# cgmb/euler

Hardware: AMD Instinct MI355X
Metric: cells*steps/sec of sim_step() (frames incl. the PCG pressure projection) + pressure-solve HBM GB/s vs roofline (higher is better)
Workload: dtype f64

## Files before the change

### euler_amd/csrc/driver.hip

```cpp
#include "euler_dev.h"
#include "k_mg.h"

#include <math.h>
#include <stdarg.h>
#include <stdlib.h>
#include <string.h>

#include <vector>

int eu_launch_build_system(euler_sim* S, float dt);
int eu_launch_velocity_update(euler_sim* S, float dt, int finish);
int eu_pressure_current(euler_sim* S);
int eu_unskew(euler_sim* S, const void* skew, void* rowmajor, int elem_bytes);
int eu_unskew_fluid(euler_sim* S, const double* skew, double* rowmajor);
double* eu_current_search_direction(euler_sim* S);
int eu_launch_tile_table(euler_sim* S);
int eu_skew(euler_sim* S, const void* rowmajor, void* skew, int elem_bytes);
int eu_set_source_count(euler_sim* S, size_t nsrc);

static thread_local char g_err[512] = "";

void eu_set_error(const char* fmt, ...) {
  va_list ap;
  va_start(ap, fmt);
// ... 105 lines not shown
  S->tile_w = w;
  return EULER_OK;
}

bool eu_resident_eligible(const euler_sim* S) {
  if (S->res_disabled || S->cfg.resident == EULER_RESIDENT_OFF) return false;
  if (S->cfg.precond != EULER_PRECOND_IC0_TILE || S->tile_w != 16 || S->cfg.sweep_mode == EULER_SWEEP_SIMPLE || S->cfg.dot_mode != EULER_DOT_TREE) return false;
  if (S->has_comm || S->slab_on || S->p2p_on) return false;
  const int cap = eu_resident_capacity(const_cast<euler_sim*>(S), S->cfg.pcg_precision == EULER_PCG_F32);
  if (S->cfg.pcg_precision == EULER_PCG_F32) return cap > 0 && S->geom.nbands * (S->geom.T / 16) <= 4 * cap;
  return cap > 0;
}
extern "C" int euler_resident_info(euler_sim* S, uint64_t out[3]) {
  if (!S || !out) return EULER_EINVAL;
  out[0] = eu_resident_eligible(S) ? 1 : 0; out[1] = S->res_solves; out[2] = S->res_fallbacks;
  return EULER_OK;
}

extern "C" int euler_set_option(euler_sim* S, int32_t key, int64_t value) {
  if (!S || key <= 0 || key >= EULER_OPT__COUNT) { eu_set_error("euler_set_option: unknown key %d", (int)key); return EULER_EINVAL; }
  bool ok = true;
  const char* when = nullptr;
  switch (key) {
    case EULER_OPT_P_STEPS: ok = value == 2 || value == 4 || value == 8; break;
    case EULER_OPT_SA_RUN: ok = value == 8 || value == 16 || value == 32;
      if (ok && value != 8 && (S->has_comm || eu_is_two_level(S))) when = "on a handle without a communicator, in the parity or the plain tile-local mode (the others run runs of 8)";
      break;
    case EULER_OPT_RCCL_SMALL: ok = value >= 0 && value <= 2; if (S->rccl) when = "before euler_set_comm_rccl"; break;
    case EULER_OPT_RCCL_NO_EXCHANGE: ok = value == 0 || value == 1; if (S->rccl) when = "before euler_set_comm_rccl"; break;
    case EULER_OPT_SLAB_FUSION: ok = value == 0 || value == 1; if (S->p2p_on) when = "before euler_p2p_connect"; break;
    case EULER_OPT_RESIDENT_CAP: case EULER_OPT_GRID4_MIN_CELLS: case EULER_OPT_RESIDENT_FORCE_TIMEOUT: ok = value >= 0; break;
    case EULER_OPT_MG_SPLIT_LEVEL: ok = value >= -1 && value < 12; break;
    case EULER_OPT_PROFILE_STRIDE: ok = value >= 1 && value <= 1024; break;
    case EULER_OPT_MG_SPLIT_ACTIVE: ok = false; break;
    case EULER_OPT_ADVECT_RK2: ok = value == 0 || value == 1;
      if (ok && value == 1 && S->slab_on) when = "on a whole-grid handle (row slabs: the midpoint samples reach one row beyond the ghost rows)";
      break;
    case EULER_OPT_ADVECT_MACCORMACK: ok = value == 0 || value == 1;
      if (ok && value == 1 && S->slab_on) when = "on a whole-grid handle (row slabs: the correction reads the forward result one row beyond the own rows)";
      break;
    default: ok = value == 0 || value == 1; break;
  }
  if (!ok) { eu_set_error("euler_set_option: key %d does not take the value %lld", (int)key, (long long)value); return EULER_EINVAL; }
  if (when) { eu_set_error("euler_set_option: key %d must be set %s", (int)key, when); return EULER_ESTATE; }
  HIPCHK(hipStreamSynchronize(S->stream));
  if (key == EULER_OPT_ADVECT_MACCORMACK && value == 1 && !S->mc_u) {
    float *a = nullptr, *b = nullptr;
    const size_t bytes = S->C * sizeof(float);
    if (eu_dalloc(S, &a, S->C, EU_MEM_HANDLE, EU_MEM_ZERO | EU_DEV_QUIET) || eu_dalloc(S, &b, S->C, EU_MEM_HANDLE, EU_MEM_ZERO | EU_DEV_QUIET)) {
      (void)eu_dev_free(S, a);
      eu_set_error("euler_set_option: EULER_OPT_ADVECT_MACCORMACK needs %zu bytes of scratch", 2 * bytes);
      return EULER_ENOMEM;
    }
    S->mc_u = a; S->mc_v = b;
  }
  if (key == EULER_OPT_P_STEPS || key == EULER_OPT_SA_RUN) {
    int rcp = eu_pressure_current(S);
    if (rcp) return rcp;
  }
  S->opt[key] = value;
  if (key == EULER_OPT_P_STEPS || key == EULER_OPT_SA_RUN) S->s_ring_n = 0;
  if (key == EULER_OPT_MG_SPLIT_LEVEL) { eu_mg_split_release(S); S->opt[EULER_OPT_MG_SPLIT_ACTIVE] = 0; }
  return EULER_OK;
}
extern "C" int euler_get_option(euler_sim* S, int32_t key, int64_t* value) {
  if (!S || !value || key <= 0 || key >= EULER_OPT__COUNT) { eu_set_error("euler_get_option: unknown key %d", (int)key); return EULER_EINVAL; }
  *value = S->opt[key];
  return EULER_OK;
}

static const char* eu_precond_combination(const euler_sim* S, int precond, int tile_w, int has_comm, int slab_on, int p2p_on) {
  const bool coarse = precond == EULER_PRECOND_IC0_TILE2 || precond == EULER_PRECOND_IC0_TILE_MG;
  if (!coarse) return nullptr;
  if (tile_w != 16 || S->cfg.sweep_mode == EULER_SWEEP_SIMPLE) return "the coarse-correction preconditioners run on tiles of 16 records with the band schedule";
  if (precond == EULER_PRECOND_IC0_TILE2 && (has_comm || slab_on)) return "EULER_PRECOND_IC0_TILE2 runs on one GPU (row slabs: EULER_PRECOND_IC0_TILE_MG)";
  if (precond == EULER_PRECOND_IC0_TILE_MG && has_comm && (!slab_on || p2p_on)) return "EULER_PRECOND_IC0_TILE_MG with several ranks: row-slab handles without mailboxes only";
  return nullptr;
}

extern "C" int euler_set_precond(euler_sim* S, int32_t precond, int32_t tile_records) {
  if (!S || precond < EULER_PRECOND_IC0 || precond > EULER_PRECOND_IC0_TILE_MG) { eu_set_error("euler_set_precond: bad argument"); return EULER_EINVAL; }
  const int w = tile_records <= 0 ? 16 : tile_records;
  if (w != 8 && w != 16 && w != 32) { eu_set_error("precond_tile_records = %d: 8, 16 or 32 (0 = 16)", tile_records); return EULER_EINVAL; }
  if (const char* why = eu_precond_combination(S, precond, w, S->has_comm, S->slab_on, S->p2p_on)) { eu_set_error("euler_set_precond: %s", why); return EULER_EINVAL; }
// ... 882 lines not shown
```

### euler_amd/csrc/euler_dev.h

```cpp
#pragma once

#include <hip/hip_runtime.h>
#include <stdint.h>
#include <stdio.h>

#include "euler.h"
#include "euler_host.h"
#include "eu_valid.h"
#include "eu_mem.h"

#define EU_H 1.0f
#define EU_RHO 1.0f
#define EU_G (-10.0f)

#define CM_FLUID 0x01
#define CM_RIGHT 0x02
#define CM_UP    0x04
#define CM_LEFT  0x08
#define CM_DOWN  0x10
#define CM_DIAG_SHIFT 5
#define CM_INTERIOR 0x9F
#define EU_CHUNK_INTERIOR 0x80000000u

enum {
  KC_TIMESTEP = 0, KC_MARKER_ADVECT, KC_MARKER_EVENTS, KC_MARKER_BIN, KC_MARKER_COMPACT, KC_SOURCES,
  KC_SELECT, KC_EXTRAPOLATE, KC_ADVECT_VELOCITY, KC_BUILD_SYSTEM, KC_PRECON_FACTOR,
  KC_FORWARD_SOLVE, KC_BACKWARD_SOLVE, KC_APPLY_A, KC_DOT, KC_UPDATE_PR, KC_UPDATE_SEARCH,
  KC_REDUCE_FINAL, KC_VELOCITY_UPDATE, KC_JACOBI, KC_MISC, KC_PRECOND_TILE, KC_COARSE_CYCLE, KC_RESIDENT, KC__COUNT
};

struct PcgScalars {
  double sigma, zs, sigma_new, alpha, beta, rnorm;
// ... 160 lines not shown
  double* cc_null;
  int mg_levels, mg_nx[12], mg_ny[12];
  size_t mg_off[12], mg_cells;
  double* mg_a;
  unsigned long long* mg_a0i;
  double *mg_rhs, *mg_x;
  double* mg_wd;
  uint8_t* mg_inner0; double mg_ic[9];
  double* mg_part;
  double* mg_dot;
  double* mg_null0;
  double* mg_m0;
  void* mg_split;
  double* mg_xbuf; int mg_xslot;
  unsigned long long* res_gran;
  unsigned long long res_tag;
  int* res_err;
  int res_disabled;
  unsigned int res_last_chunks;
  int res_have_last, res_skip_once;
  unsigned long long res_solves, res_fallbacks;
  int pcg_fields_resident;
  int tile_w;
  double* s_ring[8];
  void* s_ring_alloc[8];
  double* s_base[2];
  int s_ring_n;
  int s_launched;
  int s_none;
  int s_stale;
  const double* tile_as_override;
  double* partial2;
  struct RngJump* rng_jump;
  uint8_t* chunk_flag;
  uint8_t* chunk_prev;
  uint8_t* chunk_part;
  eu_mem mem;
  double* zhalo;
  double* zrows;
  int z_halo_last;
  double* tile_table;
  unsigned long long* chunk_bits;
  unsigned int* chunk_list;
  size_t chunk_words, chunk_cap;
  double* xrows;
  size_t xrow_len;
  int gs_cur;
  double* alpha_buf;
// ... 311 lines not shown
```

### euler_amd/csrc/k_grid.hip

```cpp
#include "k_pcg.h"
#include "k_transport.h"

#include <stdlib.h>

__device__ __forceinline__ void dt_from_maxima(MarkerState* ms, float frame_time_left, unsigned int mu_bits, unsigned int mv_bits) {
  const float mu = __uint_as_float(mu_bits), mv = __uint_as_float(mv_bits);
  const float max_distance = 0.75f * EU_H;
  const float max_velocity = sqrtf(mu + mv);
  ms->dt = fminf(max_distance / max_velocity, frame_time_left);
  ms->max_u2_bits = 0u;
  ms->max_v2_bits = 0u;
}
template <bool FUSE_DT>
__global__ __launch_bounds__(256) void k_maxsq(const float* __restrict__ u, const float* __restrict__ v,
                                               int X, int Y, MarkerState* ms, int y0, int y1, float frame_time_left) {
  float mu = 0.f, mv = 0.f;
  const bool vec = (X & 3) == 0;
  for (int yq = y0 + 4 * (int)blockIdx.x; yq < y1; yq += 4 * (int)gridDim.x) {
    if (vec) {
      for (int x = 4 * (int)threadIdx.x; x < X; x += 4 * 256) {
        float4 a[4], b[4];
#pragma unroll
        for (int r = 0; r < 4; ++r) {
          const int y = yq + r < y1 ? yq + r : y1 - 1;
// ... 651 lines not shown
    const bool f1 = count[i + 1] != 0;
    float o = 0.f;
    if (solid[i] | solid[i + 1]) o = 0.f;
    else if (f0 | f1) {
      double p1 = p[skew_index(g, x + 1, y)];
      if (f1 && p1 < 0.0) p1 = 0.0;
      o = uin[i] + (neg_inv * (float)(p1 - p0)) * dt;
    }
    uout[i] = o;
  }
  if (y < Y - 1) {
    const bool f1 = count[i + X] != 0;
    float o = 0.f;
    if (solid[i] | solid[i + X]) o = 0.f;
    else if (f0 | f1) {
      double p1 = p[skew_index(g, x, y + 1)];
      if (f1 && p1 < 0.0) p1 = 0.0;
      o = vin[i] + (neg_inv * (float)(p1 - p0)) * dt;
    }
    vout[i] = o;
  }
}

struct VuRing { const double* s[8]; int n, steps, use; };
#define VU_W 48
#define VU_ILP 4
__global__ __launch_bounds__(256) void k_velocity_update_para(const float* __restrict__ uin, const float* __restrict__ vin, float* __restrict__ uout, float* __restrict__ vout,
                                                              const double* __restrict__ p, const uint8_t* __restrict__ mask, const uint8_t* __restrict__ count,
                                                              const uint8_t* __restrict__ solid, SkewGeom g, float dt, const PcgScalars* sc, VuRing ring, MarkerState* ms,
                                                              int band_lo, int do_max, int skip_zero,
                                                              const uint8_t* __restrict__ tmap, int tnx) {
  __shared__ double sp[65][VU_W + 1];
  __shared__ float s_mu[4], s_mv[4];
  const int units = g.T / VU_W;
  const size_t blk = eu_xcd_block();
  const int band = band_lo + (int)(blk / units), t0 = (int)(blk % units) * VU_W;
  const int X = g.X, Y = g.Y, tid = threadIdx.x;
  if (skip_zero && tmap && eu_tiles_idle_cur(tmap, tnx, band, t0 > 63 ? (t0 - 63) >> 6 : 0, (t0 + VU_W - 1) >> 6, true)) return;
  int cnt = 0, from = 0;
  if (ring.use && sc->nonzero && sc->iters > 0) {
    const int n_it = sc->iters;
    from = n_it - 1 >= ring.steps ? (n_it - 1) / ring.steps * ring.steps : 0;
    cnt = n_it - from;
  }
  double al[8];
  const double* sq[8];
#pragma unroll
  for (int j = 0; j < 8; ++j) { const int it = from + (j < cnt ? j : 0); al[j] = sc->alpha_hist[it & 7]; sq[j] = ring.s[it % ring.n]; }
  const size_t ebase = ((size_t)band * g.TS + (size_t)t0) * 64;
  static_assert((64 * VU_W) % (256 * VU_ILP) == 0, "whole rounds of VU_ILP elements per thread");
  for (int c0 = tid; c0 < 64 * VU_W; c0 += 256 * VU_ILP) {
    uint8_t m[VU_ILP];
    double pv[VU_ILP];
    bool any = false;
#pragma unroll
    for (int u = 0; u < VU_ILP; ++u) { m[u] = mask[ebase + (size_t)(c0 + 256 * u)]; any = any || (m[u] & CM_FLUID); }
    if (__any(any)) {
#pragma unroll
      for (int u = 0; u < VU_ILP; ++u) pv[u] = p[ebase + (size_t)(c0 + 256 * u)];
#pragma unroll
      for (int j = 0; j < 8; ++j)
        if (j < cnt) {
          double sv[VU_ILP];
#pragma unroll
          for (int u = 0; u < VU_ILP; ++u) sv[u] = sq[j][ebase + (size_t)(c0 + 256 * u)];
#pragma unroll
          for (int u = 0; u < VU_ILP; ++u) pv[u] = pv[u] + sv[u] * al[j];
        }
    } else {
#pragma unroll
      for (int u = 0; u < VU_ILP; ++u) pv[u] = 0.0;
    }
#pragma unroll
    for (int u = 0; u < VU_ILP; ++u) {
      const int c = c0 + 256 * u;
      const double v = (m[u] & CM_FLUID) ? (pv[u] < 0.0 ? 0.0 : pv[u]) : 0.0;
      sp[(c & 127) >> 1][2 * (c >> 7) + (c & 1)] = v;
    }
  }
  {
    size_t e = 0;
    bool want = false, above = false;
    int hl = 0, hj = 0;
    if (tid < 64) { e = ebase + (size_t)VU_W * 64 + 2 * (size_t)tid; want = true; hl = tid; hj = VU_W; }
    else if (tid < 64 + VU_W) {
      const int j = tid - 64 + 1, x = t0 - 64 + j;
      hl = 64; hj = j;
      if (x >= 0 && x < X && band + 1 < g.nbands && count[(size_t)(band + 1) * 64 * X + x] != 0) { e = ((size_t)(band + 1) * g.TS + (size_t)(x & ~1)) * 64 + (size_t)(x & 1); want = true; above = true; }
    }
    if (tid < 64 + VU_W) {
      double pv = 0.0;
      if (want && (above || (mask[e] & CM_FLUID))) {
        pv = p[e];
#pragma unroll
        for (int j = 0; j < 8; ++j) if (j < cnt) pv = pv + sq[j][e] * al[j];
        pv = pv < 0.0 ? 0.0 : pv;
      }
      sp[hl][hj] = pv;
    }
  }
  __syncthreads();
  const float neg_inv = -(1.f / (EU_RHO * EU_H));
  float mu = 0.f, mv = 0.f;
  static_assert((64 * VU_W) % (256 * 4) == 0, "whole rounds of four cells per thread");
  for (int c0 = tid; c0 < 64 * VU_W; c0 += 256 * 4) {
    size_t ii[4]; bool in[4]; int ll[4], jj[4], xx[4], yy[4];
    uint8_t c_0[4], c_r[4], c_u[4], s_0[4], s_r[4], s_u[4];
    float ui[4], vi[4];
#pragma unroll
    for (int u = 0; u < 4; ++u) {
      const int c = c0 + 256 * u;
      ll[u] = c / VU_W; jj[u] = c % VU_W;
      xx[u] = t0 - ll[u] + jj[u]; yy[u] = band * 64 + ll[u];
      in[u] = xx[u] >= 0 && xx[u] < X && yy[u] < Y;
      ii[u] = (size_t)(yy[u] < Y ? yy[u] : Y - 1) * X + (size_t)(xx[u] < 0 ? 0 : xx[u] >= X ? X - 1 : xx[u]);
      const bool hr = in[u] && xx[u] < X - 1, hu = in[u] && yy[u] < Y - 1;
      c_0[u] = count[ii[u]]; s_0[u] = solid[ii[u]];
      c_r[u] = count[ii[u] + (hr ? 1 : 0)]; s_r[u] = solid[ii[u] + (hr ? 1 : 0)];
// ... 90 lines not shown
           S->solid, S->b, S->r, S->p, S->q, S->z, S->cellmask, S->sc, S->geom, dt, S->e_lo, S->e_cnt, S->chunk_flag, S->chunk_part, S->chunk_prev);
  eu_vd_assembled(&S->vd);
  LAUNCH(S, KC_BUILD_SYSTEM, k_pack_chunk_bits, dim3(eu_blocks(S->chunk_words, 256)), dim3(256), S->chunk_flag, S->chunk_bits, S->chunk_words, S->chunk_cap);
  int rc = eu_ordered_select(S, S->chunk_bits, S->chunk_words, S->chunk_list, &S->sc->n_chunks);
  if (rc) return rc;
  const bool no_interior = S->opt[EULER_OPT_NO_INTERIOR] != 0;
  if (!no_interior)
    LAUNCH(S, KC_BUILD_SYSTEM, k_mark_interior, dim3(eu_blocks(S->chunk_cap, 256)), dim3(256), S->chunk_list, S->sc, S->chunk_part);
  return eu_launch_band_ranges(S);
}

int eu_pressure_current(euler_sim* S) {
  const int mode = eu_vd_pressure_owes(&S->vd);
  if (!mode) return EULER_OK;
  eu_vd_pressure_made_current(&S->vd);
  if (mode == 1) { int rc = eu_launch_finish_p(S); if (rc) return rc; }
  LAUNCH(S, KC_VELOCITY_UPDATE, k_clamp_p, dim3(eu_blocks(S->e_cnt, 256 * 4, 4096)), dim3(256), S->p, S->cellmask, S->e_lo, S->e_cnt);
  return EULER_OK;
}
int eu_launch_velocity_update(euler_sim* S, float dt, int finish) {
  const bool one_pass = (!S->has_comm || S->slab_on) && S->opt[EULER_OPT_VELOCITY_TWO_PASS] == 0 && (!S->slab_on || !finish);
  if (one_pass) {
    VuRing ring;
    for (int k = 0; k < 8; ++k) ring.s[k] = S->s_ring[k < S->s_ring_n ? k : 0];
    ring.n = S->s_ring_n > 0 ? S->s_ring_n : 1; ring.steps = ring.n; ring.use = finish && S->s_ring_n > 0;
    if (!ring.use) for (int k = 0; k < 8; ++k) ring.s[k] = S->p;
    const int do_max = S->slab_on ? 0 : 1;
    if (eu_vd_update_clears_maxima(&S->vd, do_max)) HIPCHK(hipMemsetAsync(&S->ms->max_u2_bits, 0, 2 * sizeof(unsigned int), S->stream));
    LAUNCH(S, KC_VELOCITY_UPDATE, k_velocity_update_para, dim3((unsigned)((size_t)(S->band_hi - S->band_lo) * (S->geom.T / VU_W))), dim3(256), S->utmp, S->vtmp, S->u, S->v, S->p, S->cellmask,
           S->count, S->solid, S->geom, dt, S->sc, ring, S->ms, S->band_lo, do_max, eu_vd_update_skips_zeros(&S->vd, S->slab_on),
           eu_tile_map_on(S) ? (const uint8_t*)S->tmap : (const uint8_t*)nullptr, S->tmap_nx);
    eu_vd_velocity_updated(&S->vd, 1, ring.use, do_max);
    return EULER_OK;
  }
  if (finish) { int rc = eu_launch_finish_p(S); if (rc) return rc; }
  dim3 grid((S->X + 63) / 64, (S->row_hi - S->row_lo + 3) / 4);
  LAUNCH(S, KC_VELOCITY_UPDATE, k_velocity_update, grid, dim3(256), S->utmp, S->vtmp, S->u, S->v, S->p, S->count,
         S->solid, S->geom, dt, S->row_lo, S->row_hi);
  eu_vd_velocity_updated(&S->vd, 0, 0, 0);
  return EULER_OK;
}

template <typename T>
__global__ __launch_bounds__(256) void k_unskew(const T* __restrict__ skew, T* __restrict__ rowmajor, SkewGeom g, int y0, int y1) {
  const size_t i = (size_t)blockIdx.x * blockDim.x + threadIdx.x;
  if (i < (size_t)g.X * (y1 - y0)) rowmajor[i] = skew[skew_index(g, (int)(i % g.X), y0 + (int)(i / g.X))];
}
template <typename T>
__global__ __launch_bounds__(256) void k_skew(const T* __restrict__ rowmajor, T* __restrict__ skew, SkewGeom g, int y0, int y1) {
// ... 28 lines not shown
```

### euler_amd/csrc/k_pcg.h

```cpp
#pragma once

#include "euler_dev.h"
#include "k_mg.h"

#define COMM_CALL(expr) do { if ((expr) != 0) { eu_set_error("communicator callback failed: %s", #expr); return EULER_ECOMM; } } while (0)
#define LOC(ptr) ((ptr) + S->e_lo)
enum { SW_FACTOR = 0, SW_FORWARD = 1, SW_BACKWARD = 2 };

int eu_launch_build_system(euler_sim* S, float dt);
int eu_launch_velocity_update(euler_sim* S, float dt, int finish);
int eu_launch_band_ranges(euler_sim* S);
int eu_launch_sweep(euler_sim* S, int op, int cls, int force, int fin_qq = -1);
int eu_launch_factor_tile(euler_sim* S, int force);
int eu_launch_precond_tile(euler_sim* S, int rupd, int sweeps, int fin_dot, int force, double alpha, bool r_only = false, int zform = -1);
int eu_launch_search_apply(euler_sim* S, int it);
int eu_launch_finish_p(euler_sim* S);
int eu_launch_dot(euler_sim* S, const double* a, const double* b, int fin_op, int force);
int eu_comm_exchange(euler_sim* S, double* send_lo, double* send_hi, double* recv_lo, double* recv_hi, int count, double* small, int nsmall);
int eu_comm_finish(euler_sim* S, int fin_op, int is_max, int force);
int eu_comm_halo_two(euler_sim* S, double* a, double* b);
bool tile_recompute(const euler_sim* S);
int p_steps(const euler_sim* S);

enum { FIN_SIGMA_INIT = 0, FIN_ALPHA, FIN_RNORM, FIN_BETA, FIN_STORE_ONLY, FIN_TO_COMM };
// ... 125 lines not shown
    const double qv = t * cpre;
    const double res = (cm & CM_FLUID) ? qv : 0.0;
    const double carry = -1.0 * cpre * res;
    own = carry; out = carry;
    if (j & 1) zz[j >> 1].y = res; else zz[j >> 1].x = res;
  }
  own = 0.0; out = 0.0;
#pragma unroll
  for (int j = W - 1; j >= 0; --j) {
    const int cm = (int)((mm[j >> 1] >> ((j & 1) * 8)) & 0xff);
    const double cin = (j & 1) ? zz[j >> 1].y : zz[j >> 1].x, cpre = (j & 1) ? pp[j >> 1].y : pp[j >> 1].x;
    const double nbv = wave_shift_inject<DPP_WAVE_SHL1>(out, 0.0);
    const double kr = ((cm & CM_RIGHT) ? -1.0 : 0.0) * cpre, ku = ((cm & CM_UP) ? -1.0 : 0.0) * cpre;
    const double t = cin - kr * own - ku * nbv;
    const double zv = t * cpre;
    const double res = (cm & CM_FLUID) ? zv : 0.0;
    own = res; out = res;
    if (DOT && (cm & CM_FLUID)) dsum += res * ((j & 1) ? rr[j >> 1].y : rr[j >> 1].x);
    if (j & 1) zz[j >> 1].y = res; else zz[j >> 1].x = res;
  }
}
struct ZrArgs { const double* r; const double* pre; const double* table; const double* halo; const double* rows; int X; };
struct CoarseRef { const double* y; int shift, nx, ny, band0; };
struct SaHist { const double* s[6]; };

struct SweepArgs {
  SkewGeom g;
  const uint8_t* mask;
  const unsigned int* fbits_fwd;
  const unsigned int* fbits_bwd;
  int fb_stride;
  double* pre;
  const double* in;
  double* out;
  unsigned long long* granules;
  int gran_stride;
  const unsigned long long* xg_in;
  unsigned long long* xg_out;
  const int4* ranges;
  int band_lo, nb_local;
  int couple;
  unsigned int* ticket;
  unsigned int ticket_base;
  unsigned int epoch;
  const PcgScalars* sc;
  int force;
  int* error;
// ... 60 lines not shown
```

### euler_amd/csrc/k_pcg.hip

```cpp
#include "k_pcg.h"

#include <cmath>
#include <vector>

template <bool IS_MAX>
__global__ __launch_bounds__(RED_THREADS) void k_reduce_final(const double* __restrict__ partial, int n, PcgScalars* sc,
                                                              int op, int force) {
  if (!force && pcg_idle(sc)) return;
  double v = 0.0;
  for (int i = threadIdx.x; i < n; i += RED_THREADS) {
    const double w = partial[i];
    if (IS_MAX) v = w > v ? w : v; else v += w;
  }
  v = IS_MAX ? block_max(v) : block_sum(v);
  if (threadIdx.x == 0) pcg_scalar_step(sc, op, v);
}

template <bool EDGES>
__global__ __launch_bounds__(RED_THREADS) void k_dot_partial(const double* __restrict__ a, const double* __restrict__ b,
                                                             const uint8_t* __restrict__ mask, size_t S,
                                                             double* __restrict__ partial, PcgScalars* sc, int force,
                                                             unsigned int* counter, int fin_op, int TS, int nb_local, int edges) {
  if (!force && pcg_idle(sc)) return;
  const size_t chunk = (((S + gridDim.x - 1) / gridDim.x) + 1) & ~(size_t)1;
// ... 183 lines not shown
  }
}

__global__ __launch_bounds__(256) void k_publish_edge_rows(double* arr, SkewGeom g, int y0, int y1, const PcgScalars* sc) {
  if (pcg_idle(sc)) return;
  const int x = blockIdx.x * 256 + threadIdx.x;
  if (x >= g.X) return;
  const int y = blockIdx.y == 0 ? y0 : y1;
  if (y < 0) return;
  double* p = arr + skew_index(g, x, y);
  st_system(p, *p);
}

__global__ __launch_bounds__(256) void k_jacobi(const double* __restrict__ r, double* __restrict__ z,
                                                const uint8_t* __restrict__ mask, size_t S, const PcgScalars* sc, int force) {
  if (!force && pcg_idle(sc)) return;
  for (size_t i = (size_t)blockIdx.x * blockDim.x + threadIdx.x; i < S; i += (size_t)gridDim.x * blockDim.x) {
    const uint8_t m = mask[i];
    const int d = m >> CM_DIAG_SHIFT;
    z[i] = (m & CM_FLUID) ? r[i] / (double)(d ? d : 1) : 0.0;
  }
}

struct SRing { const double* s[8]; int n, steps; };
__global__ __launch_bounds__(256) void k_finish_p(double* __restrict__ p, const uint8_t* __restrict__ mask, size_t e_lo, size_t S,
                                                  const PcgScalars* sc, SRing ring) {
  if (!sc->nonzero || sc->iters == 0) return;
  const int n_it = sc->iters;
  const int from = n_it - 1 >= ring.steps ? (n_it - 1) / ring.steps * ring.steps : 0;
  const int cnt = n_it - from;
  double al[8];
  const double* sp[8];
#pragma unroll
  for (int j = 0; j < 8; ++j) { const int it = from + (j < cnt ? j : 0); al[j] = sc->alpha_hist[it & 7]; sp[j] = ring.s[it % ring.n] + e_lo; }
  for (size_t i = 2 * ((size_t)blockIdx.x * blockDim.x + threadIdx.x); i < S; i += 2 * (size_t)gridDim.x * blockDim.x) {
    const unsigned int mm = *reinterpret_cast<const unsigned short*>(mask + i);
    const bool f0 = (mm & CM_FLUID) != 0, f1 = ((mm >> 8) & CM_FLUID) != 0;
    if (!(f0 | f1)) continue;
    sw_d2 pv = *reinterpret_cast<const sw_d2*>(p + i);
#pragma unroll
    for (int j = 0; j < 8; ++j) {
      if (j < cnt) {
        const sw_d2 sv = *reinterpret_cast<const sw_d2*>(sp[j] + i);
        if (f0) pv.x = pv.x + sv.x * al[j];
        if (f1) pv.y = pv.y + sv.y * al[j];
      }
    }
    *reinterpret_cast<sw_d2*>(p + i) = pv;
  }
}

int eu_launch_finish_p(euler_sim* S) {
  if (S->s_ring_n <= 0) return EULER_OK;
  SRing ring;
  for (int k = 0; k < 8; ++k) ring.s[k] = S->s_ring[k < S->s_ring_n ? k : 0];
  ring.n = S->s_ring_n; ring.steps = S->s_ring_n;
  LAUNCH(S, KC_UPDATE_PR, k_finish_p, dim3(eu_blocks(S->e_cnt, 256 * 4, 4096)), dim3(256), S->p + S->e_lo, S->cellmask + S->e_lo, S->e_lo, S->e_cnt, S->sc, ring);
  return EULER_OK;
}

__global__ void k_scalar_epilogue(PcgScalars* sc, int op, int force) {
  if (!force && pcg_idle(sc)) return;
  pcg_scalar_step(sc, op, sc->comm_val);
}
__global__ void k_nonzero_to_comm(PcgScalars* sc) { sc->comm_val = sc->nonzero ? 1.0 : 0.0; }
__global__ void k_nonzero_from_comm(PcgScalars* sc) { sc->nonzero = sc->comm_val != 0.0; }

__global__ __launch_bounds__(256) void k_pack_row(const double* __restrict__ skew, double* __restrict__ row, SkewGeom g, int band, int lane) {
  const int x = blockIdx.x * 256 + threadIdx.x;
  if (x < g.X) row[x] = skew[skew_index(g, x, band * 64 + lane)];
}
__global__ __launch_bounds__(256) void k_unpack_row(double* __restrict__ skew, const double* __restrict__ row, SkewGeom g, int band, int lane) {
  const int x = blockIdx.x * 256 + threadIdx.x;
  if (x < g.X) skew[skew_index(g, x, band * 64 + lane)] = row[x];
}

template <bool PACK>
__global__ __launch_bounds__(256) void k_halo_rows2(double* a, double* b, double* lo, double* hi, SkewGeom g, int band_lo, int band_hi,
// ... 119 lines not shown
    const bool coarse = eu_is_two_level(S);
    if (S->band_lo > 0) {
      HIPCHK(hipMemcpyAsync(xrow(S, XR_GS_LO0), xrow(S, XR_ZRECV_LO), (size_t)X * 8, hipMemcpyDeviceToDevice, S->stream));
      if (coarse) { int rc = eu_launch_coarse_add_row(S, xrow(S, XR_GS_LO0), 64 * S->band_lo - 1); if (rc) return rc; }
      hipLaunchKernelGGL(k_unpack_row, dim3(nbk), dim3(256), 0, S->stream, S->s, xrow(S, XR_GS_LO0), S->geom, S->band_lo - 1, 63);
    }
    if (S->band_hi < S->geom.nbands) {
      HIPCHK(hipMemcpyAsync(xrow(S, XR_GS_HI0), xrow(S, XR_ZRECV_HI), (size_t)X * 8, hipMemcpyDeviceToDevice, S->stream));
      if (coarse) { int rc = eu_launch_coarse_add_row(S, xrow(S, XR_GS_HI0), 64 * S->band_hi); if (rc) return rc; }
      hipLaunchKernelGGL(k_unpack_row, dim3(nbk), dim3(256), 0, S->stream, S->s, xrow(S, XR_GS_HI0), S->geom, S->band_hi, 0);
    }
    S->gs_cur = 0;
  } else if (S->has_comm) { int rc = comm_halo_s(S); if (rc) return rc; }
  SkewGeom gl = S->geom;
  gl.S = S->e_cnt;
  double* out = tile_fused(S) ? S->q : S->z;
  LAUNCH(S, KC_APPLY_A, k_apply_a, dim3(loc_red_blocks(S)), dim3(RED_THREADS), LOC(S->s), LOC(out), LOC(S->cellmask), gl,
         S->partial, S->sc, force, S->red_counter, seq ? -1 : fin_or_comm(S, FIN_ALPHA));
  if (seq)
    LAUNCH(S, KC_DOT, k_dot_sequential, dim3(1), dim3(256), out, S->s, S->cellmask, S->geom, S->sc, (int)FIN_ALPHA, force);
  return S->has_comm ? eu_comm_finish(S, FIN_ALPHA, 0, force) : EULER_OK;
}

int p_steps(const euler_sim* S) {
  if (S->p2p_on || sa_run(S) != 8) return 2;
  return (int)S->opt[EULER_OPT_P_STEPS];
}
static int ring_begin(euler_sim* S) {
  const int n = p_steps(S);
  if (!S->s_base[0]) { S->s_base[0] = S->s; S->s_base[1] = S->s2; }
  if (n > 2) { S->s = S->s_base[0]; S->s2 = S->s_base[1]; }
  else if (S->s != S->s_base[0] && S->s != S->s_base[1]) { S->s = S->s_base[0]; S->s2 = S->s_base[1]; }
  else if (S->s2 != S->s_base[0] && S->s2 != S->s_base[1]) S->s2 = S->s == S->s_base[0] ? S->s_base[1] : S->s_base[0];
  S->s_ring[0] = S->s; S->s_ring[1] = S->s2;
  for (int k = 2; k < n; ++k) {
    if (!S->s_ring_alloc[k]) {
      const size_t elems = S->Sw + EU_SKEW_SLACK;
      if (eu_dev_alloc(S, &S->s_ring_alloc[k], elems * sizeof(double), EU_MEM_RING, EU_DEV_QUIET)) {
        eu_dev_free_group(S, EU_MEM_RING);
        for (void*& d : S->s_ring_alloc) d = nullptr;
        S->opt[EULER_OPT_P_STEPS] = 2;
        return ring_begin(S);
      }
      HIPCHK(hipMemsetAsync(S->s_ring_alloc[k], 0, elems * sizeof(double), S->stream));
    }
    S->s_ring[k] = static_cast<double*>(S->s_ring_alloc[k]) + EU_SKEW_SLACK - S->skew_off;
  }
  S->s_ring_n = n;
  S->s_launched = 0;
  return EULER_OK;
}
double* eu_current_search_direction(euler_sim* S) {
  if (S->s_ring_n < 2 || S->s_launched <= 0) return S->s;
  (void)hipStreamSynchronize(S->stream);
  const int ran = S->sc_host->nonzero ? S->sc_host->iters : 0;
  if (ran <= 0 || ran > S->s_launched) return S->s;
  return S->s_ring[(ran - 1) % S->s_ring_n];
}

__global__ void k_pcg_reset(PcgScalars* sc, double tol, int max_iters) {
  sc->sigma = sc->zs = sc->sigma_new = sc->alpha = sc->alpha_prev = sc->beta = sc->rnorm = 0.0;
  sc->tol = tol; sc->nonzero = 0; sc->done = 0; sc->iters = 0; sc->max_iters = max_iters; sc->zfix = 0;
}

static inline bool first_direction_folded(const euler_sim* S) { return tile_fused(S) && eu_is_mg(S) && !S->has_comm && S->cfg.dot_mode != EULER_DOT_SEQUENTIAL && sa_run(S) == 8; }
struct Solve {
  PcgScalars prev;
  int pred_iters;
  bool drain_poll;
// ... 242 lines not shown
```

### euler_amd/csrc/k_search.hip

```cpp
#include "k_pcg.h"

#include <type_traits>

#define SA_THREADS 256
struct SaPair { sw_d2 z, so; double ez0, es0, ez1, es1; };

__device__ __forceinline__ double pick3(int t, int tb1, int tb2, double v0, double v1, double v2) {
  double v = v0;
  v = t >= tb1 ? v1 : v;
  v = t >= tb2 ? v2 : v;
  return v;
}
template <int SLAB, int PMODE, int SA_RUN, int COARSE = 0, bool STORE = true, bool ZR = false>
__global__ __launch_bounds__(SA_THREADS, (COARSE == 2 && PMODE == 1 && SLAB == 0) ? 4 : 1) void k_search_apply(const double* __restrict__ s_old, const double* __restrict__ z,
                                                             double* __restrict__ s_new, double* __restrict__ out,
                                                             const uint8_t* __restrict__ mask, SkewGeom g,
                                                             double* __restrict__ partial, PcgScalars* sc, int force,
                                                             unsigned int* counter, int fin_op, SlabNeighbours nbr,
                                                             double* __restrict__ p, double* s_new_base, double* s_old_base,
                                                             const unsigned int* __restrict__ chunk_list,
                                                             CoarseRef cref, SaHist hist, ZrArgs zr) {
  static_assert(PMODE == 1 || PMODE == 2 || PMODE == 4 || PMODE == 8, "PMODE: p is left alone (1) or takes the N fmadds that are due (the ring's length)");
  static_assert(!ZR || (SLAB == 0 && SA_RUN == 8 && COARSE == 0), "ZR: one GPU, runs of one tile, no coarse part");
  __shared__ double s_cy[COARSE == 2 ? SA_THREADS / 64 : 1][COARSE == 2 ? MG_NI + 1 : 1][64];
  __shared__ double s_ce[COARSE == 2 ? SA_THREADS / 64 : 1][COARSE == 2 ? MG_NI + 1 : 1][64];
  if (!force && pcg_idle(sc)) return;
  __shared__ sw_d2 s_ztab[ZR ? 8 : 1][64];
  if (ZR) {
    for (int k = threadIdx.x; k < 8 * 64; k += SA_THREADS) (&s_ztab[0][0])[k] = reinterpret_cast<const sw_d2*>(zr.table)[k];
    __syncthreads();
  }
  const double beta = sc->beta;
  (void)s_new_base; (void)s_old_base;
  constexpr int NPA = PMODE >= 2 ? PMODE : 2;
  double al[NPA] = {};
  if (PMODE >= 2) {
    const int k = sc->iters;
#pragma unroll
    for (int j = 0; j < NPA; ++j) al[j] = sc->alpha_hist[(k - NPA + j) & 7];
  }
  const int lane = threadIdx.x & 63;
  const int TS = g.TS, npairs = TS / 2;
  const int nb_local = (int)(g.S / ((size_t)TS * 64));
  const int cpb = (npairs + SA_RUN - 1) / SA_RUN, total = nb_local * cpb;
  const int n_waves = gridDim.x * (SA_THREADS / 64);
  const bool edge_lane = lane == 0 || lane == 63;
  double t = 0.0;
  const bool listed = chunk_list != nullptr;
  const int ntb16 = g.T / 16;
  const int todo = listed ? (int)sc->n_chunks : total;
  typedef std::integral_constant<bool, true> yes_t;
  typedef std::integral_constant<bool, false> no_t;
  for (int i = blockIdx.x * (SA_THREADS / 64) + (threadIdx.x >> 6); i < todo; i += n_waves) {
    int c = i, per = cpb;
    bool interior = false;
    if (listed) { const unsigned int ent = chunk_list[i]; interior = (ent & EU_CHUNK_INTERIOR) != 0; c = (int)(ent & ~EU_CHUNK_INTERIOR); per = ntb16; }
    const int lb = c / per, P0 = (c % per) * SA_RUN, P1 = ZR ? P0 + SA_RUN : (P0 + SA_RUN < npairs ? P0 + SA_RUN : npairs);
    const size_t bbase = (size_t)lb * TS * 64 + 2 * lane;
    auto run = [&](auto full_tag) {
      constexpr bool FULL = decltype(full_tag)::value;
      unsigned int mm[SA_RUN];
      unsigned int any = 0;
#pragma unroll
// ... 132 lines not shown
      double prev_y = sprime(A).y;
      sw_d2 cur = sprime(B);
#pragma unroll
      for (int j = 0; j < SA_RUN; ++j) {
        const int P = P0 + j;
        if (P < P1) {
          SaPair D;
          load_pair(P + 2 <= P1 ? P + 2 : -1, D, j + 2 < SA_RUN ? mm[j + 2] : 0u);
          const unsigned int m0 = mm[j] & 0xff, m1 = mm[j] >> 8;
          const sw_d2 nxt = sprime(Cn);
          const double e0 = B.ez0 + beta * B.es0, e1 = B.ez1 + beta * B.es1;
          if (SLAB == 2 && ghost && edge_lane) {
            if ((mm[j] & CM_FLUID) && (mm[j] & vbit)) gsn[2 * P + gcol] = e0;
            if (((mm[j] >> 8) & CM_FLUID) && ((mm[j] >> 8) & vbit)) gsn[2 * P + 1 + gcol] = e1;
          }
          const double dn0 = wave_shift_inject<DPP_WAVE_SHR1>(prev_y, e0), up0 = wave_shift_inject<DPP_WAVE_SHL1>(cur.y, e0);
          const double dn1 = wave_shift_inject<DPP_WAVE_SHR1>(cur.x, e1), up1 = wave_shift_inject<DPP_WAVE_SHL1>(nxt.x, e1);
          if ((m0 | m1) & CM_FLUID) {
            const size_t i = bbase + (size_t)P * 128;
            sw_d2 cc = B.so, o = {0.0, 0.0};
            if (PMODE >= 2) {
              sw_d2 pv = *reinterpret_cast<const sw_d2*>(p + i);
              constexpr int NP = PMODE >= 2 ? PMODE : 2;
              sw_d2 sv[NP];
              sv[0] = *reinterpret_cast<const sw_d2*>(s_new + i);
#pragma unroll
              for (int j = 1; j < NP - 1; ++j) sv[j] = *reinterpret_cast<const sw_d2*>(hist.s[j - 1] + i);
              sv[NP - 1] = B.so;
#pragma unroll
              for (int j = 0; j < NP; ++j) {
                if (m0 & CM_FLUID) pv.x = pv.x + sv[j].x * al[j];
                if (m1 & CM_FLUID) pv.y = pv.y + sv[j].y * al[j];
              }
              *reinterpret_cast<sw_d2*>(p + i) = pv;
            }
            if (m0 & CM_FLUID) cc.x = cur.x;
            if (m1 & CM_FLUID) cc.y = cur.y;
            if (m0 & CM_FLUID) {
              double v = (double)(int)(m0 >> CM_DIAG_SHIFT) * cc.x;
              v = v - ((m0 & CM_RIGHT) ? cc.y : 0.0);
              v = v - ((m0 & CM_UP) ? up0 : 0.0);
              v = v - ((m0 & CM_LEFT) ? prev_y : 0.0);
              v = v - ((m0 & CM_DOWN) ? dn0 : 0.0);
              o.x = v;
              t += v * cc.x;
            }
            if (m1 & CM_FLUID) {
              double v = (double)(int)(m1 >> CM_DIAG_SHIFT) * cc.y;
// ... 29 lines not shown
  if (fin_op >= 0) block_finish<false, SA_THREADS>(t, partial, counter, sc, fin_op);
}

static inline unsigned sa_blocks(const euler_sim* S, int run) {
  return eu_blocks((size_t)(S->band_hi - S->band_lo) * ((S->geom.TS / 2 + run - 1) / run), SA_THREADS / 64, 2048);
}
struct SaCall { SkewGeom gl; int fin; SlabNeighbours nbr; CoarseRef cref; SaHist hist; ZrArgs zr; };
template <int SLAB, int PMODE, int RUN, int COARSE, bool STORE, bool ZR = false>
static void sa_launch(euler_sim* S, const SaCall& c) {
  LAUNCH(S, KC_APPLY_A, (k_search_apply<SLAB, PMODE, RUN, COARSE, STORE, ZR>), dim3(sa_blocks(S, RUN)), dim3(SA_THREADS), LOC(S->s), LOC(S->z), LOC(S->s2),
         LOC(S->q), LOC(S->cellmask), c.gl, S->partial, S->sc, 0, S->red_counter, c.fin, c.nbr, LOC(S->p), S->s2, S->s, RUN == 8 ? S->chunk_list : (const unsigned int*)nullptr, c.cref, c.hist, c.zr);
}
template <int SLAB, int COARSE, int PMODE>
static void sa_pick_run(euler_sim* S, const SaCall& c, int run, bool store) {
  if constexpr (COARSE == 0 && SLAB != 2 && PMODE <= 2) {
    if constexpr (SLAB == 0) { if (run == 16) return sa_launch<SLAB, PMODE, 16, COARSE, true>(S, c); }
    if (run != 8) return sa_launch<SLAB, PMODE, 32, COARSE, true>(S, c);
  }
  if (store) sa_launch<SLAB, PMODE, 8, COARSE, true>(S, c); else sa_launch<SLAB, PMODE, 8, COARSE, false>(S, c);
}
template <int SLAB, int COARSE>
static void sa_pick(euler_sim* S, const SaCall& c, int pmode, int run, bool store) {
  if constexpr (SLAB != 1) {
    if (pmode == 8) return sa_pick_run<SLAB, COARSE, 8>(S, c, run, store);
    if (pmode == 4) return sa_pick_run<SLAB, COARSE, 4>(S, c, run, store);
  }
  if (pmode == 2) sa_pick_run<SLAB, COARSE, 2>(S, c, run, store); else sa_pick_run<SLAB, COARSE, 1>(S, c, run, store);
}
int eu_launch_search_apply(euler_sim* S, int it) {
  const bool seq = S->cfg.dot_mode == EULER_DOT_SEQUENTIAL && !S->has_comm;
  SlabNeighbours nbr = {nullptr, nullptr, nullptr, nullptr, S->band_hi - S->band_lo, nullptr, nullptr, nullptr, nullptr, nullptr, nullptr};
  const bool direct = S->has_comm && eu_p2p_has_neighbour_arrays(S);
  const bool ghost = ghost_mode(S);
  if (ghost) {
    const int c = S->gs_cur;
    if (S->band_lo > 0) { nbr.zrow_dn = xrow(S, XR_ZRECV_LO); nbr.srow_dn = xrow(S, XR_GS_LO0 + c); nbr.snew_dn = xrow(S, XR_GS_LO0 + (c ^ 1)); }
    if (S->band_hi < S->geom.nbands) { nbr.zrow_up = xrow(S, XR_ZRECV_HI); nbr.srow_up = xrow(S, XR_GS_HI0 + c); nbr.snew_up = xrow(S, XR_GS_HI0 + (c ^ 1)); }
    S->gs_cur = c ^ 1;
  } else if (direct) {
    eu_p2p_neighbour_arrays(S, &nbr.z_dn, &nbr.s_dn, &nbr.z_up, &nbr.s_up);
    if (nbr.z_dn) { nbr.z_dn += S->e_lo; nbr.s_dn += S->e_lo; }
    if (nbr.z_up) { nbr.z_up += S->e_lo; nbr.s_up += S->e_lo; }
  } else if (S->has_comm) {
    if (int rc = eu_comm_halo_two(S, S->z, S->s)) return rc;
  }
  const int steps = S->s_ring_n;
  const int pmode = (it >= steps && it % steps == 0) ? steps : 1;
  const bool mg = eu_is_mg(S);
  SaCall c = {S->geom, S->has_comm ? fin_or_comm(S, FIN_ALPHA) : (seq ? -1 : (int)FIN_ALPHA), nbr,
              {mg ? S->mg_x : S->cc_y, mg ? 0 : S->coarse_shift, mg ? S->mg_nx[0] : S->coarse_nx, mg ? S->mg_ny[0] : S->coarse_ny, S->band_lo},
              {{nullptr, nullptr, nullptr, nullptr, nullptr, nullptr}}, {S->r, S->precon, S->tile_table, S->zhalo, S->zrows, S->X}};
  c.gl.S = S->e_cnt;
  for (int j = 1; j + 1 < steps; ++j) c.hist.s[j - 1] = LOC(S->s_ring[j]);
  const int run = sa_run(S);
  const bool store = !tile_recompute(S);
  const bool coarse = eu_is_two_level(S) && tile_fused(S);
  if (S->z_halo_last) sa_launch<0, 1, 8, 0, false, true>(S, c);
  else if (coarse && ghost) sa_pick<2, 2>(S, c, pmode, run, store);
  else if (coarse && mg) sa_pick<0, 2>(S, c, pmode, run, store);
  else if (coarse) sa_pick<0, 1>(S, c, pmode, run, store);
  else if (ghost) sa_pick<2, 0>(S, c, pmode, run, store);
  else if (direct) sa_pick<1, 0>(S, c, pmode, run, store);
  else sa_pick<0, 0>(S, c, pmode, run, store);
  S->s = S->s_ring[it % steps]; S->s2 = S->s_ring[(it + 1) % steps];
  S->s_launched = it + 1;
  if (seq) eu_launch_dot(S, S->q, S->s, FIN_ALPHA, 0);
  return S->has_comm ? eu_comm_finish(S, FIN_ALPHA, 0, 0) : EULER_OK;
}
```

Measured before the change: 199.4 million.

## Deepen the deferred p-update search-direction ring to 16 or 32 slots on large grids

Extends the ring of stored search directions from at most 8 to up to 32 entries, so the pressure vector p is updated in batches of up to 32 directions instead of 8. Alphas older than the 8-entry history are copied into a new alpha_old buffer. The depth is chosen automatically from free memory on single-GPU grids of at least 2^24 cells. This cuts how often p is read and written during PCG, at the cost of extra ring memory and wider gather loops in the search-apply, finish and velocity-update kernels.

```diff
diff --git a/euler_amd/csrc/driver.hip b/euler_amd/csrc/driver.hip
--- a/euler_amd/csrc/driver.hip
+++ b/euler_amd/csrc/driver.hip
@@ -151,7 +151,7 @@
   bool ok = true;
   const char* when = nullptr;
   switch (key) {
-    case EULER_OPT_P_STEPS: ok = value == 2 || value == 4 || value == 8; break;
+    case EULER_OPT_P_STEPS: ok = eu_ring_depth_ok(value) != 0; break;
     case EULER_OPT_SA_RUN: ok = value == 8 || value == 16 || value == 32;
       if (ok && value != 8 && (S->has_comm || eu_is_two_level(S))) when = "on a handle without a communicator, in the parity or the plain tile-local mode (the others run runs of 8)";
       break;
@@ -188,7 +188,8 @@
     if (rcp) return rcp;
   }
   S->opt[key] = value;
-  if (key == EULER_OPT_P_STEPS || key == EULER_OPT_SA_RUN) S->s_ring_n = 0;
+  if (key == EULER_OPT_P_STEPS || key == EULER_OPT_SA_RUN) { S->s_ring_n = 0; S->p_depth = 0; }
+  if (key == EULER_OPT_P_STEPS) S->p_pinned = 1;
   if (key == EULER_OPT_MG_SPLIT_LEVEL) { eu_mg_split_release(S); S->opt[EULER_OPT_MG_SPLIT_ACTIVE] = 0; }
   return EULER_OK;
 }
diff --git a/euler_amd/csrc/eu_ring.h b/euler_amd/csrc/eu_ring.h
--- /dev/null
+++ b/euler_amd/csrc/eu_ring.h
@@ -0,0 +1,20 @@
+#ifndef EU_RING_H
+#define EU_RING_H
+
+#if defined(__HIPCC__) || defined(__CUDACC__)
+#define EU_RING_FN __host__ __device__ static inline
+#else
+#define EU_RING_FN static inline
+#endif
+
+#define EU_RING_MAX 32
+#define EU_ALPHA_OLD 32
+
+EU_RING_FN int eu_ring_depth_ok(long long n) { return n == 2 || n == 4 || n == 8 || n == 16 || n == 32; }
+EU_RING_FN int eu_ring_step_down(int n) { return n > 2 ? n / 2 : 2; }
+EU_RING_FN int eu_alpha_copy_due(int k) { return k >= 8 && (k & 7) == 0; }
+EU_RING_FN int eu_alpha_in_hist(int it, int iters) { return it >= iters - 8; }
+EU_RING_FN int eu_ring_finish_from(int iters, int steps) { return iters - 1 >= steps ? (iters - 1) / steps * steps : 0; }
+EU_RING_FN int eu_ring_pmode(int it, int steps) { return (it >= steps && it % steps == 0) ? steps : 1; }
+
+#endif
diff --git a/euler_amd/csrc/euler_dev.h b/euler_amd/csrc/euler_dev.h
--- a/euler_amd/csrc/euler_dev.h
+++ b/euler_amd/csrc/euler_dev.h
@@ -8,6 +8,7 @@
 #include "euler_host.h"
 #include "eu_valid.h"
 #include "eu_mem.h"
+#include "eu_ring.h"
 
 #define EU_H 1.0f
 #define EU_RHO 1.0f
@@ -214,8 +215,11 @@
   unsigned long long res_solves, res_fallbacks;
   int pcg_fields_resident;
   int tile_w;
-  double* s_ring[8];
-  void* s_ring_alloc[8];
+  double* s_ring[EU_RING_MAX];
+  void* s_ring_alloc[EU_RING_MAX];
+  double* alpha_old;
+  int p_pinned;
+  int p_depth;
   double* s_base[2];
   int s_ring_n;
   int s_launched;
diff --git a/euler_amd/csrc/k_grid.hip b/euler_amd/csrc/k_grid.hip
--- a/euler_amd/csrc/k_grid.hip
+++ b/euler_amd/csrc/k_grid.hip
@@ -697,7 +697,7 @@
   }
 }
 
-struct VuRing { const double* s[8]; int n, steps, use; };
+struct VuRing { const double* s[EU_RING_MAX]; const double* alpha_old; int n, steps, use; };
 #define VU_W 48
 #define VU_ILP 4
 __global__ __launch_bounds__(256) void k_velocity_update_para(const float* __restrict__ uin, const float* __restrict__ vin, float* __restrict__ uout, float* __restrict__ vout,
@@ -712,16 +712,13 @@
   const int band = band_lo + (int)(blk / units), t0 = (int)(blk % units) * VU_W;
   const int X = g.X, Y = g.Y, tid = threadIdx.x;
   if (skip_zero && tmap && eu_tiles_idle_cur(tmap, tnx, band, t0 > 63 ? (t0 - 63) >> 6 : 0, (t0 + VU_W - 1) >> 6, true)) return;
-  int cnt = 0, from = 0;
+  int cnt = 0, from = 0, n_it = 0;
   if (ring.use && sc->nonzero && sc->iters > 0) {
-    const int n_it = sc->iters;
-    from = n_it - 1 >= ring.steps ? (n_it - 1) / ring.steps * ring.steps : 0;
+    n_it = sc->iters;
+    from = eu_ring_finish_from(n_it, ring.steps);
     cnt = n_it - from;
   }
-  double al[8];
-  const double* sq[8];
-#pragma unroll
-  for (int j = 0; j < 8; ++j) { const int it = from + (j < cnt ? j : 0); al[j] = sc->alpha_hist[it & 7]; sq[j] = ring.s[it % ring.n]; }
+  auto alpha_of = [&](int it) __attribute__((always_inline)) { return eu_alpha_in_hist(it, n_it) ? sc->alpha_hist[it & 7] : ring.alpha_old[it & (EU_ALPHA_OLD - 1)]; };
   const size_t ebase = ((size_t)band * g.TS + (size_t)t0) * 64;
   static_assert((64 * VU_W) % (256 * VU_ILP) == 0, "whole rounds of VU_ILP elements per thread");
   for (int c0 = tid; c0 < 64 * VU_W; c0 += 256 * VU_ILP) {
@@ -733,15 +730,19 @@
     if (__any(any)) {
 #pragma unroll
       for (int u = 0; u < VU_ILP; ++u) pv[u] = p[ebase + (size_t)(c0 + 256 * u)];
-#pragma unroll
-      for (int j = 0; j < 8; ++j)
-        if (j < cnt) {
-          double sv[VU_ILP];
-#pragma unroll
-          for (int u = 0; u < VU_ILP; ++u) sv[u] = sq[j][ebase + (size_t)(c0 + 256 * u)];
-#pragma unroll
-          for (int u = 0; u < VU_ILP; ++u) pv[u] = pv[u] + sv[u] * al[j];
-        }
+      for (int g0 = 0; g0 < cnt; g0 += 8) {
+#pragma unroll
+        for (int j = 0; j < 8; ++j)
+          if (g0 + j < cnt) {
+            const double a = alpha_of(from + g0 + j);
+            const double* sq = ring.s[g0 + j];
+            double sv[VU_ILP];
+#pragma unroll
+            for (int u = 0; u < VU_ILP; ++u) sv[u] = sq[ebase + (size_t)(c0 + 256 * u)];
+#pragma unroll
+            for (int u = 0; u < VU_ILP; ++u) pv[u] = pv[u] + sv[u] * a;
+          }
+      }
     } else {
 #pragma unroll
       for (int u = 0; u < VU_ILP; ++u) pv[u] = 0.0;
@@ -767,8 +768,13 @@
       double pv = 0.0;
       if (want && (above || (mask[e] & CM_FLUID))) {
         pv = p[e];
-#pragma unroll
-        for (int j = 0; j < 8; ++j) if (j < cnt) pv = pv + sq[j][e] * al[j];
+        for (int g0 = 0; g0 < cnt; g0 += 8) {
+          double sv[8];
+#pragma unroll
+          for (int j = 0; j < 8; ++j) if (g0 + j < cnt) sv[j] = ring.s[g0 + j][e];
+#pragma unroll
+          for (int j = 0; j < 8; ++j) if (g0 + j < cnt) pv = pv + sv[j] * alpha_of(from + g0 + j);
+        }
         pv = pv < 0.0 ? 0.0 : pv;
       }
       sp[hl][hj] = pv;
@@ -905,9 +911,10 @@
   const bool one_pass = (!S->has_comm || S->slab_on) && S->opt[EULER_OPT_VELOCITY_TWO_PASS] == 0 && (!S->slab_on || !finish);
   if (one_pass) {
     VuRing ring;
-    for (int k = 0; k < 8; ++k) ring.s[k] = S->s_ring[k < S->s_ring_n ? k : 0];
+    for (int k = 0; k < EU_RING_MAX; ++k) ring.s[k] = S->s_ring[k < S->s_ring_n ? k : 0];
     ring.n = S->s_ring_n > 0 ? S->s_ring_n : 1; ring.steps = ring.n; ring.use = finish && S->s_ring_n > 0;
-    if (!ring.use) for (int k = 0; k < 8; ++k) ring.s[k] = S->p;
+    ring.alpha_old = S->s_ring_n > 8 ? S->alpha_old : nullptr;
+    if (!ring.use) for (int k = 0; k < EU_RING_MAX; ++k) ring.s[k] = S->p;
     const int do_max = S->slab_on ? 0 : 1;
     if (eu_vd_update_clears_maxima(&S->vd, do_max)) HIPCHK(hipMemsetAsync(&S->ms->max_u2_bits, 0, 2 * sizeof(unsigned int), S->stream));
     LAUNCH(S, KC_VELOCITY_UPDATE, k_velocity_update_para, dim3((unsigned)((size_t)(S->band_hi - S->band_lo) * (S->geom.T / VU_W))), dim3(256), S->utmp, S->vtmp, S->u, S->v, S->p, S->cellmask,
diff --git a/euler_amd/csrc/k_pcg.h b/euler_amd/csrc/k_pcg.h
--- a/euler_amd/csrc/k_pcg.h
+++ b/euler_amd/csrc/k_pcg.h
@@ -171,7 +171,7 @@
 }
 struct ZrArgs { const double* r; const double* pre; const double* table; const double* halo; const double* rows; int X; };
 struct CoarseRef { const double* y; int shift, nx, ny, band0; };
-struct SaHist { const double* s[6]; };
+struct SaHist { const double* s[6]; const double* l0; const double* early[EU_RING_MAX - 8]; const double* alpha_old; double* acopy; int groups; };
 
 struct SweepArgs {
   SkewGeom g;
diff --git a/euler_amd/csrc/k_pcg.hip b/euler_amd/csrc/k_pcg.hip
--- a/euler_amd/csrc/k_pcg.hip
+++ b/euler_amd/csrc/k_pcg.hip
@@ -229,28 +229,33 @@
   }
 }
 
-struct SRing { const double* s[8]; int n, steps; };
+struct SRing { const double* s[EU_RING_MAX]; const double* alpha_old; int n, steps; };
 __global__ __launch_bounds__(256) void k_finish_p(double* __restrict__ p, const uint8_t* __restrict__ mask, size_t e_lo, size_t S,
                                                   const PcgScalars* sc, SRing ring) {
   if (!sc->nonzero || sc->iters == 0) return;
   const int n_it = sc->iters;
-  const int from = n_it - 1 >= ring.steps ? (n_it - 1) / ring.steps * ring.steps : 0;
+  const int from = eu_ring_finish_from(n_it, ring.steps);
   const int cnt = n_it - from;
-  double al[8];
-  const double* sp[8];
-#pragma unroll
-  for (int j = 0; j < 8; ++j) { const int it = from + (j < cnt ? j : 0); al[j] = sc->alpha_hist[it & 7]; sp[j] = ring.s[it % ring.n] + e_lo; }
   for (size_t i = 2 * ((size_t)blockIdx.x * blockDim.x + threadIdx.x); i < S; i += 2 * (size_t)gridDim.x * blockDim.x) {
     const unsigned int mm = *reinterpret_cast<const unsigned short*>(mask + i);
     const bool f0 = (mm & CM_FLUID) != 0, f1 = ((mm >> 8) & CM_FLUID) != 0;
     if (!(f0 | f1)) continue;
     sw_d2 pv = *reinterpret_cast<const sw_d2*>(p + i);
+    for (int g0 = 0; g0 < cnt; g0 += 8) {
+      sw_d2 sv[8];
+      double al[8];
 #pragma unroll
-    for (int j = 0; j < 8; ++j) {
-      if (j < cnt) {
-        const sw_d2 sv = *reinterpret_cast<const sw_d2*>(sp[j] + i);
-        if (f0) pv.x = pv.x + sv.x * al[j];
-        if (f1) pv.y = pv.y + sv.y * al[j];
+      for (int j = 0; j < 8; ++j) {
+        const int it = from + (g0 + j < cnt ? g0 + j : g0);
+        al[j] = eu_alpha_in_hist(it, n_it) ? sc->alpha_hist[it & 7] : ring.alpha_old[it & (EU_ALPHA_OLD - 1)];
+        if (g0 + j < cnt) sv[j] = *reinterpret_cast<const sw_d2*>(ring.s[it - from] + e_lo + i);
+      }
+#pragma unroll
+      for (int j = 0; j < 8; ++j) {
+        if (g0 + j < cnt) {
+          if (f0) pv.x = pv.x + sv[j].x * al[j];
+          if (f1) pv.y = pv.y + sv[j].y * al[j];
+        }
       }
     }
     *reinterpret_cast<sw_d2*>(p + i) = pv;
@@ -260,7 +265,8 @@
 int eu_launch_finish_p(euler_sim* S) {
   if (S->s_ring_n <= 0) return EULER_OK;
   SRing ring;
-  for (int k = 0; k < 8; ++k) ring.s[k] = S->s_ring[k < S->s_ring_n ? k : 0];
+  for (int k = 0; k < EU_RING_MAX; ++k) ring.s[k] = S->s_ring[k < S->s_ring_n ? k : 0];
+  ring.alpha_old = S->s_ring_n > 8 ? S->alpha_old : nullptr;
   ring.n = S->s_ring_n; ring.steps = S->s_ring_n;
   LAUNCH(S, KC_UPDATE_PR, k_finish_p, dim3(eu_blocks(S->e_cnt, 256 * 4, 4096)), dim3(256), S->p + S->e_lo, S->cellmask + S->e_lo, S->e_lo, S->e_cnt, S->sc, ring);
   return EULER_OK;
@@ -426,29 +432,48 @@
   return S->has_comm ? eu_comm_finish(S, FIN_ALPHA, 0, force) : EULER_OK;
 }
 
+#define EU_RING_DEEP_MIN_CELLS (1ll << 24)
+static int ring_depth_choose(const euler_sim* S) {
+  if (S->has_comm || S->slab_on || (long long)S->X * S->Y < EU_RING_DEEP_MIN_CELLS) return 8;
+  size_t free_b = 0, total_b = 0;
+  if (hipMemGetInfo(&free_b, &total_b) != hipSuccess) { (void)hipGetLastError(); return 8; }
+  const size_t per = (S->Sw + EU_SKEW_SLACK) * sizeof(double);
+  for (int n = EU_RING_MAX; n > 8; n /= 2) {
+    size_t need = EU_ALPHA_OLD * sizeof(double);
+    for (int k = 2; k < n; ++k) if (!S->s_ring_alloc[k]) need += per;
+    if (need <= free_b / 2) return n;
+  }
+  return 8;
+}
 int p_steps(const euler_sim* S) {
   if (S->p2p_on || sa_run(S) != 8) return 2;
-  return (int)S->opt[EULER_OPT_P_STEPS];
+  return S->p_depth ? S->p_depth : (int)S->opt[EULER_OPT_P_STEPS];
 }
 static int ring_begin(euler_sim* S) {
+  if (!S->p_depth && !S->p_pinned && !S->p2p_on && sa_run(S) == 8) S->p_depth = ring_depth_choose(S);
   const int n = p_steps(S);
   if (!S->s_base[0]) { S->s_base[0] = S->s; S->s_base[1] = S->s2; }
   if (n > 2) { S->s = S->s_base[0]; S->s2 = S->s_base[1]; }
   else if (S->s != S->s_base[0] && S->s != S->s_base[1]) { S->s = S->s_base[0]; S->s2 = S->s_base[1]; }
   else if (S->s2 != S->s_base[0] && S->s2 != S->s_base[1]) S->s2 = S->s == S->s_base[0] ? S->s_base[1] : S->s_base[0];
   S->s_ring[0] = S->s; S->s_ring[1] = S->s2;
-  for (int k = 2; k < n; ++k) {
-    if (!S->s_ring_alloc[k]) {
-      const size_t elems = S->Sw + EU_SKEW_SLACK;
-      if (eu_dev_alloc(S, &S->s_ring_alloc[k], elems * sizeof(double), EU_MEM_RING, EU_DEV_QUIET)) {
+  for (int k = 2; k <= n; ++k) {
+    const bool alphas = k == n;
+    if (alphas ? (n > 8 && !S->alpha_old) : !S->s_ring_alloc[k]) {
+      const size_t elems = alphas ? (size_t)EU_ALPHA_OLD : S->Sw + EU_SKEW_SLACK;
+      void* blk = nullptr;
+      if (eu_dev_alloc(S, &blk, elems * sizeof(double), EU_MEM_RING, EU_DEV_QUIET)) {
         eu_dev_free_group(S, EU_MEM_RING);
         for (void*& d : S->s_ring_alloc) d = nullptr;
-        S->opt[EULER_OPT_P_STEPS] = 2;
+        S->alpha_old = nullptr;
+        S->p_depth = eu_ring_step_down(n);
+        if (S->p_pinned) S->opt[EULER_OPT_P_STEPS] = S->p_depth;
         return ring_begin(S);
       }
-      HIPCHK(hipMemsetAsync(S->s_ring_alloc[k], 0, elems * sizeof(double), S->stream));
-    }
-    S->s_ring[k] = static_cast<double*>(S->s_ring_alloc[k]) + EU_SKEW_SLACK - S->skew_off;
+      HIPCHK(hipMemsetAsync(blk, 0, elems * sizeof(double), S->stream));
+      if (alphas) S->alpha_old = static_cast<double*>(blk); else S->s_ring_alloc[k] = blk;
+    }
+    if (!alphas) S->s_ring[k] = static_cast<double*>(S->s_ring_alloc[k]) + EU_SKEW_SLACK - S->skew_off;
   }
   S->s_ring_n = n;
   S->s_launched = 0;
diff --git a/euler_amd/csrc/k_search.hip b/euler_amd/csrc/k_search.hip
--- a/euler_amd/csrc/k_search.hip
+++ b/euler_amd/csrc/k_search.hip
@@ -3,6 +3,7 @@
 #include <type_traits>
 
 #define SA_THREADS 256
+typedef __attribute__((address_space(4))) double ConstDouble;
 struct SaPair { sw_d2 z, so; double ez0, es0, ez1, es1; };
 
 __device__ __forceinline__ double pick3(int t, int tb1, int tb2, double v0, double v1, double v2) {
@@ -34,11 +35,16 @@
   (void)s_new_base; (void)s_old_base;
   constexpr int NPA = PMODE >= 2 ? PMODE : 2;
   double al[NPA] = {};
+  int k_it = 0, early_groups = 0;
+  (void)k_it; (void)early_groups;
   if (PMODE >= 2) {
     const int k = sc->iters;
+    k_it = k;
+    if (PMODE == 8) early_groups = hist.groups - 1;
 #pragma unroll
     for (int j = 0; j < NPA; ++j) al[j] = sc->alpha_hist[(k - NPA + j) & 7];
   }
+  if (hist.acopy && blockIdx.x == 0 && threadIdx.x < 8) hist.acopy[((sc->iters - 8) & (EU_ALPHA_OLD - 8)) + threadIdx.x]       = sc->alpha_hist[threadIdx.x];
   const int lane = threadIdx.x & 63;
   const int TS = g.TS, npairs = TS / 2;
   const int nb_local = (int)(g.S / ((size_t)TS * 64));
@@ -217,8 +223,28 @@
             if (PMODE >= 2) {
               sw_d2 pv = *reinterpret_cast<const sw_d2*>(p + i);
               constexpr int NP = PMODE >= 2 ? PMODE : 2;
+              if (PMODE == 8) {
+                constexpr int EG = COARSE == 2 ? (SLAB == 2 ? 2 : 4) : 8;
+                const int early_terms = 8 * early_groups;
+#pragma clang loop unroll(disable)
+                for (int t0 = 0; t0 < early_terms; t0 += EG) {
+                  const ConstDouble* ao = (const ConstDouble*)hist.alpha_old + ((k_it - 8 - early_terms + t0) & (EU_ALPHA_OLD - 1));
+                  sw_d2 ev[EG];
+#pragma unroll
+                  for (int j = 0; j < EG; ++j) {
+                    const double* src = (j == 0 && t0 == 0) ? s_new : hist.early[t0 + j];
+                    ev[j] = *reinterpret_cast<const sw_d2*>(src + i);
+                  }
+#pragma unroll
+                  for (int j = 0; j < EG; ++j) {
+                    const double a = ao[j];
+                    if (m0 & CM_FLUID) pv.x = pv.x + ev[j].x * a;
+                    if (m1 & CM_FLUID) pv.y = pv.y + ev[j].y * a;
+                  }
+                }
+              }
               sw_d2 sv[NP];
-              sv[0] = *reinterpret_cast<const sw_d2*>(s_new + i);
+              sv[0] = *reinterpret_cast<const sw_d2*>((PMODE == 8 && early_groups > 0 ? hist.l0 : s_new) + i);
 #pragma unroll
               for (int j = 1; j < NP - 1; ++j) sv[j] = *reinterpret_cast<const sw_d2*>(hist.s[j - 1] + i);
               sv[NP - 1] = B.so;
@@ -294,7 +320,7 @@
 template <int SLAB, int COARSE>
 static void sa_pick(euler_sim* S, const SaCall& c, int pmode, int run, bool store) {
   if constexpr (SLAB != 1) {
-    if (pmode == 8) return sa_pick_run<SLAB, COARSE, 8>(S, c, run, store);
+    if (pmode >= 8) return sa_pick_run<SLAB, COARSE, 8>(S, c, run, store);
     if (pmode == 4) return sa_pick_run<SLAB, COARSE, 4>(S, c, run, store);
   }
   if (pmode == 2) sa_pick_run<SLAB, COARSE, 2>(S, c, run, store); else sa_pick_run<SLAB, COARSE, 1>(S, c, run, store);
@@ -317,13 +343,21 @@
     if (int rc = eu_comm_halo_two(S, S->z, S->s)) return rc;
   }
   const int steps = S->s_ring_n;
-  const int pmode = (it >= steps && it % steps == 0) ? steps : 1;
+  const int pmode = eu_ring_pmode(it, steps);
   const bool mg = eu_is_mg(S);
   SaCall c = {S->geom, S->has_comm ? fin_or_comm(S, FIN_ALPHA) : (seq ? -1 : (int)FIN_ALPHA), nbr,
               {mg ? S->mg_x : S->cc_y, mg ? 0 : S->coarse_shift, mg ? S->mg_nx[0] : S->coarse_nx, mg ? S->mg_ny[0] : S->coarse_ny, S->band_lo},
-              {{nullptr, nullptr, nullptr, nullptr, nullptr, nullptr}}, {S->r, S->precon, S->tile_table, S->zhalo, S->zrows, S->X}};
+              SaHist{}, {S->r, S->precon, S->tile_table, S->zhalo, S->zrows, S->X}};
   c.gl.S = S->e_cnt;
-  for (int j = 1; j + 1 < steps; ++j) c.hist.s[j - 1] = LOC(S->s_ring[j]);
+  const int early = steps > 8 ? steps - 8 : 0;
+  c.hist.groups = early / 8 + 1;
+  for (int j = 1; j + 1 < steps - early; ++j) c.hist.s[j - 1] = LOC(S->s_ring[early + j]);
+  if (early) {
+    c.hist.l0 = LOC(S->s_ring[early]);
+    for (int t = 1; t < early; ++t) c.hist.early[t] = LOC(S->s_ring[t]);
+    c.hist.alpha_old = S->alpha_old;
+    if (eu_alpha_copy_due(it)) c.hist.acopy = S->alpha_old;
+  }
   const int run = sa_run(S);
   const bool store = !tile_recompute(S);
   const bool coarse = eu_is_two_level(S) && tile_fused(S);
```

Result: slower. 195.5 million (-1.9%).
